# AI-multimodal/RankAAE

Hardware: AMD Instinct MI355X
Metric: training steps/sec (batch=256, 256-pt spectra) (higher is better)
Workload: dtype f32; 1 GPU; BASELINE configs[1]: 7000x256 synthetic spectra (7000 per GPU; train split 4900), batch 256/GPU, ae_form=compact, nstyle=6, n_aux=5, AdamW, 5 phases incl. smoothness; global_batch=256, parallelism=dp1, hip_graph=True, rng=philox tape (device), rccl_ranks=1

## Files before the change

### rankaae_amd/csrc/raae_common.h

```cpp
#pragma once
#include <hip/hip_runtime.h>
#include <stdint.h>
#include "../../include/rankaae_hip.h"

#define RAAE_WAVE 64

#define RAAE_CHECK_ARG(cond) do { if (!(cond)) return RAAE_EINVAL; } while (0)
#define RAAE_LAUNCH_RET() do { hipError_t e_ = hipGetLastError(); return (int)e_; } while (0)

typedef float f32x4 __attribute__((ext_vector_type(4)));

#ifdef RAAE_STAMPS
extern __device__ long long d_stamps[4][3][16];
extern __device__ unsigned long long d_stage_sum[4][3][16], d_stage_cnt[4][3][16];
extern __device__ long long d_stage_prev[4];
extern __device__ unsigned long long d_kind_sum[8][4][16], d_kind_cnt[8][4][16];
#endif
namespace raae {

__device__ __forceinline__ float wave_sum(float v) {
#pragma unroll
    for (int o = 32; o > 0; o >>= 1) v += __shfl_xor(v, o, 64);
    return v;
}
__device__ __forceinline__ double wave_sum(double v) {
#pragma unroll
    for (int o = 32; o > 0; o >>= 1) v += __shfl_xor(v, o, 64);
    return v;
}
__device__ __forceinline__ int wave_sum(int v) {
#pragma unroll
    for (int o = 32; o > 0; o >>= 1) v += __shfl_xor(v, o, 64);
    return v;
}

__device__ __forceinline__ double block_sum(double v, double* sh) {
    v = wave_sum(v);
    const int w = threadIdx.x >> 6, nw = (blockDim.x + 63) >> 6;
    __syncthreads();
    if ((threadIdx.x & 63) == 0) sh[w] = v;
    __syncthreads();
    double t = 0.0;
    for (int i = 0; i < nw; ++i) t += sh[i];
    return t;
}

__device__ __forceinline__ float prelu(float x, float a) { return x > 0.f ? x : a * x; }

__device__ __forceinline__ float softplus2(float x) {
    const float bx = 2.f * x;
    return bx > 20.f ? x : 0.5f * log1pf(expf(bx));
}

__device__ __forceinline__ void reduce_partials(const double* partials, int nparts, int C, double* tot_s,
                                                double* tot_q) {
    __shared__ double scr_s[256], scr_q[256];
    int Cp = 1;
    while (Cp < C) Cp <<= 1;
    const int J = 256 / Cp;
    const int t = threadIdx.x;
    if (t < 256) {
        const int c = t & (Cp - 1), j = t / Cp;
        double s = 0.0, q = 0.0;
        if (c < C) {
            const double2* p = reinterpret_cast<const double2*>(partials) + c;
            int i = j;
            for (; i + 3 * J < nparts; i += 4 * J) {
                const double2 v0 = p[(size_t)i * C], v1 = p[(size_t)(i + J) * C];
                const double2 v2 = p[(size_t)(i + 2 * J) * C], v3 = p[(size_t)(i + 3 * J) * C];
// ... 344 lines not shown
```

### rankaae_amd/csrc/raae_disc.hip

```cpp
#include "raae_common.h"
#include <stdlib.h>

namespace {

constexpr int DH = 64;
constexpr int DT = 16;
constexpr int DNS = 16;
constexpr int AP = DH + 1;

struct DiscArgs {
    const float* z_real; const float* styles; const float* noise; float sigma;
    const float* m1; const float* m2;
    const float* w1; const float* b1; const float* s1;
    const float* w2; const float* b2; const float* s2;
    const float* w3; const float* b3;
    const float* alpha;
    int n_real, n_fake, ns;
    float* dw1; float* db1; float* ds1; float* dw2; float* db2; float* ds2; float* dw3; float* db3;
    long slab_stride;
    float* dstyles;
    double* partial; unsigned* ticket; float* loss;
};

__device__ __forceinline__ double softplus_dd(double x) { return x > 0.0 ? x + log1p(exp(-x)) : log1p(exp(x)); }

template <bool MM>
__device__ __forceinline__ void disc_fused_body(const DiscArgs& a) {
    __shared__ float W1[DH * DNS], W2[DH * (DH + 1)], W3[DH], B1[DH], B2[DH], S1[DH], S2[DH];
    __shared__ float X[DT * DNS], Z1[DT * AP], A1[DT * AP], Z2[DT * AP], A2[DT * AP], G2[DT * AP], G1[DT * AP];
    __shared__ float DL[DT];
    __shared__ double shd[16];
    __shared__ unsigned s_last;
    const int t = threadIdx.x, ns = a.ns, n = a.n_real + a.n_fake;
    for (int i = t; i < DH * DNS; i += 256) { const int o = i / DNS, k = i - o * DNS; W1[i] = k < ns ? a.w1[o * ns + k] : 0.f; }
    for (int i = t; i < DH * DH; i += 256) { const int o = i >> 6, k = i & 63; W2[o * (DH + 1) + k] = a.w2[i]; }
    if (t < DH) { W3[t] = a.w3[t]; B1[t] = a.b1[t]; B2[t] = a.b2[t]; S1[t] = a.s1[t]; S2[t] = a.s2[t]; }
    const float b3 = a.b3[0];
    const float neg_alpha = -a.alpha[0];
    float aw2[16], aw1[4];
    f32x4 mw2[4];
#pragma unroll
    for (int i = 0; i < 4; ++i) mw2[i] = (f32x4){0.f, 0.f, 0.f, 0.f};
    const int lane = t & 63, wave = t >> 6, l15 = lane & 15, l4 = lane >> 4;
#pragma unroll
    for (int i = 0; i < 16; ++i) aw2[i] = 0.f;
#pragma unroll
    for (int i = 0; i < 4; ++i) aw1[i] = 0.f;
    float ab1 = 0.f, ab2 = 0.f, as1 = 0.f, as2 = 0.f, aw3 = 0.f, ab3 = 0.f;
    double lacc = 0.0;
    const int ntiles = (n + DT - 1) / DT;
    const int r4 = t >> 4, c4 = (t & 15) * 4;
    const int wo = t >> 2, wk = (t & 3) * 16;
    __syncthreads();
    for (int tile = blockIdx.x; tile < ntiles; tile += gridDim.x) {
        const int row0 = tile * DT;
        float m1v[4] = {1.f, 1.f, 1.f, 1.f}, m2v[4] = {1.f, 1.f, 1.f, 1.f};
        if (row0 + r4 < n) {
            if (a.m1) { const float4 v = *reinterpret_cast<const float4*>(a.m1 + (size_t)(row0 + r4) * DH + c4); m1v[0] = v.x; m1v[1] = v.y; m1v[2] = v.z; m1v[3] = v.w; }
            if (a.m2) { const float4 v = *reinterpret_cast<const float4*>(a.m2 + (size_t)(row0 + r4) * DH + c4); m2v[0] = v.x; m2v[1] = v.y; m2v[2] = v.z; m2v[3] = v.w; }
        }
        for (int i = t; i < DT * DNS; i += 256) {
            const int r = i / DNS, k = i - r * DNS, row = row0 + r;
            float v = 0.f;
            if (row < n && k < ns) {
                v = row < a.n_real ? a.z_real[(size_t)row * ns + k] : a.styles[(size_t)(row - a.n_real) * ns + k];
                if (a.noise) v += a.sigma * a.noise[(size_t)row * ns + k];
            }
            X[i] = v;
        }
        __syncthreads();
        {
            const int row = row0 + r4;
#pragma unroll
            for (int j = 0; j < 4; ++j) {
                const int o = c4 + j;
                float acc = B1[o];
                for (int k = 0; k < ns; ++k) acc = fmaf(X[r4 * DNS + k], W1[o * DNS + k], acc);
                Z1[r4 * AP + o] = acc;
                float v = acc > 0.f ? acc : acc * S1[o];
                v *= m1v[j];
                A1[r4 * AP + o] = row < n ? v : 0.f;
            }
        }
        __syncthreads();
        {
            const int row = row0 + r4;
            float acc[4] = {B2[c4], B2[c4 + 1], B2[c4 + 2], B2[c4 + 3]};
            if constexpr (MM) {
                f32x4 c = {0.f, 0.f, 0.f, 0.f};
                const float* pa = A1 + l15 * AP + l4;
                const float* pb = W2 + (16 * wave + l15) * (DH + 1) + l4;
#pragma unroll
                for (int q = 0; q < DH / 4; ++q) c = __builtin_amdgcn_mfma_f32_16x16x4f32(pa[4 * q], pb[4 * q], c, 0, 0, 0);
#pragma unroll
                for (int j = 0; j < 4; ++j) Z2[(4 * l4 + j) * AP + 16 * wave + l15] = c[j];
                __syncthreads();
#pragma unroll
                for (int j = 0; j < 4; ++j) acc[j] += Z2[r4 * AP + c4 + j];
            } else {
#pragma unroll 4
                for (int k = 0; k < DH; ++k) {
                    const float x = A1[r4 * AP + k];
#pragma unroll
                    for (int j = 0; j < 4; ++j) acc[j] = fmaf(x, W2[(c4 + j) * (DH + 1) + k], acc[j]);
                }
            }
#pragma unroll
            for (int j = 0; j < 4; ++j) {
                const int o = c4 + j;
                Z2[r4 * AP + o] = acc[j];
                float v = acc[j] > 0.f ? acc[j] : acc[j] * S2[o];
                v *= m2v[j];
                A2[r4 * AP + o] = row < n ? v : 0.f;
            }
        }
        __syncthreads();
        {
            float p = 0.f;
#pragma unroll
            for (int j = 0; j < 4; ++j) p = fmaf(A2[r4 * AP + c4 + j], W3[c4 + j], p);
            p += __shfl_xor(p, 1, 64); p += __shfl_xor(p, 2, 64); p += __shfl_xor(p, 4, 64); p += __shfl_xor(p, 8, 64);
            const int row = row0 + r4;
            if ((t & 15) == 0) {
                float d = 0.f;
                if (row < n) {
                    const float o = p + b3;
                    const float sg = 1.f / (1.f + expf(-o));
                    if (row < a.n_real) { lacc += softplus_dd(-(double)o) / (double)a.n_real; d = (sg - 1.f) / (float)a.n_real; }
                    else { lacc += softplus_dd((double)o) / (double)a.n_fake; d = sg / (float)a.n_fake; }
                }
                DL[r4] = d;
            }
        }
        __syncthreads();
        {
            const float d = DL[r4];
#pragma unroll
            for (int j = 0; j < 4; ++j) {
                const int o = c4 + j;
                float g = d * W3[o];
                g *= m2v[j];
                const float z = Z2[r4 * AP + o];
                G2[r4 * AP + o] = z > 0.f ? g : g * S2[o];
                Z2[r4 * AP + o] = z > 0.f ? 0.f : g * z;
            }
        }
        __syncthreads();
        if (t < DH) {
            float w = 0.f, b = 0.f, s = 0.f;
#pragma unroll 4
            for (int r = 0; r < DT; ++r) { w = fmaf(A2[r * AP + t], DL[r], w); b += G2[r * AP + t]; s += Z2[r * AP + t]; }
            aw3 += w; ab2 += b; as2 += s;
        }
        if (t == 64) { float b = 0.f; for (int r = 0; r < DT; ++r) b += DL[r]; ab3 += b; }
        if constexpr (MM) {
#pragma unroll
            for (int q = 0; q < DT / 4; ++q) {
                const float ga = G2[(4 * q + l4) * AP + 16 * wave + l15];
#pragma unroll
                for (int tk = 0; tk < 4; ++tk)
                    mw2[tk] = __builtin_amdgcn_mfma_f32_16x16x4f32(ga, A1[(4 * q + l4) * AP + 16 * tk + l15], mw2[tk], 0, 0, 0);
            }
        } else {
#pragma unroll 2
            for (int r = 0; r < DT; ++r) {
                const float g = G2[r * AP + wo];
#pragma unroll
                for (int j = 0; j < 16; ++j) aw2[j] = fmaf(g, A1[r * AP + wk + j], aw2[j]);
            }
        }
        {
            float acc[4] = {0.f, 0.f, 0.f, 0.f};
            if constexpr (MM) {
                f32x4 c = {0.f, 0.f, 0.f, 0.f};
                const float* pa = G2 + l15 * AP + l4;
                const float* pb = W2 + l4 * (DH + 1) + 16 * wave + l15;
#pragma unroll
                for (int q = 0; q < DH / 4; ++q)
                    c = __builtin_amdgcn_mfma_f32_16x16x4f32(pa[4 * q], pb[4 * q * (DH + 1)], c, 0, 0, 0);
#pragma unroll
                for (int j = 0; j < 4; ++j) G1[(4 * l4 + j) * AP + 16 * wave + l15] = c[j];
                __syncthreads();
#pragma unroll
                for (int j = 0; j < 4; ++j) acc[j] = G1[r4 * AP + c4 + j];
            } else {
#pragma unroll 4
                for (int o = 0; o < DH; ++o) {
                    const float g = G2[r4 * AP + o];
#pragma unroll
                    for (int j = 0; j < 4; ++j) acc[j] = fmaf(g, W2[o * (DH + 1) + c4 + j], acc[j]);
                }
            }
            __syncthreads();
#pragma unroll
            for (int j = 0; j < 4; ++j) {
                const int k = c4 + j;
                float g = acc[j];
                g *= m1v[j];
                const float z = Z1[r4 * AP + k];
                G1[r4 * AP + k] = z > 0.f ? g : g * S1[k];
                Z1[r4 * AP + k] = z > 0.f ? 0.f : g * z;
            }
        }
        __syncthreads();
        if (t < DH) {
            float b = 0.f, s = 0.f;
            for (int r = 0; r < DT; ++r) { b += G1[r * AP + t]; s += Z1[r * AP + t]; }
            ab1 += b; as1 += s;
        }
#pragma unroll
        for (int j = 0; j < 4; ++j) {
            const int idx = t + 256 * j;
            if (idx < DH * ns) {
                const int o = idx / ns, k = idx - o * ns;
                float w = 0.f;
#pragma unroll 4
                for (int r = 0; r < DT; ++r) w = fmaf(G1[r * AP + o], X[r * DNS + k], w);
                aw1[j] += w;
            }
        }
        for (int i = t; i < DT * ns; i += 256) {
            const int r = i / ns, k = i - r * ns, row = row0 + r;
            if (row >= a.n_real && row < n) {
                float d = 0.f;
#pragma unroll 4
                for (int o = 0; o < DH; ++o) d = fmaf(G1[r * AP + o], W1[o * DNS + k], d);
                a.dstyles[(size_t)(row - a.n_real) * ns + k] = neg_alpha * d;
            }
        }
        __syncthreads();
    }
    const size_t slab = (size_t)blockIdx.x * (size_t)a.slab_stride;
    if constexpr (MM) {
#pragma unroll
        for (int tk = 0; tk < 4; ++tk)
#pragma unroll
            for (int j = 0; j < 4; ++j) a.dw2[slab + (16 * wave + 4 * l4 + j) * DH + 16 * tk + l15] = mw2[tk][j];
    } else {
#pragma unroll
        for (int j = 0; j < 16; ++j) a.dw2[slab + wo * DH + wk + j] = aw2[j];
    }
#pragma unroll
    for (int j = 0; j < 4; ++j) { const int idx = t + 256 * j; if (idx < DH * ns) a.dw1[slab + idx] = aw1[j]; }
    if (t < DH) {
        a.db1[slab + t] = ab1; a.ds1[slab + t] = as1; a.db2[slab + t] = ab2; a.ds2[slab + t] = as2; a.dw3[slab + t] = aw3;
    }
    if (t == 64) a.db3[slab] = ab3;
    const double tot = raae::block_sum(lacc, shd);
    if (t == 0) {
        a.partial[blockIdx.x] = tot;
        __threadfence();
        s_last = atomicAdd(a.ticket, 1u) == gridDim.x - 1 ? 1u : 0u;
    }
    __syncthreads();
    if (s_last) {
        __threadfence();
        double sum = 0.0;
        for (unsigned i = t; i < gridDim.x; i += 256) sum += ((volatile double*)a.partial)[i];
        sum = raae::block_sum(sum, shd);
        if (t == 0) {
            a.loss[0] = (float)sum;
            *a.ticket = 0u;
        }
    }
}
template <bool MM>
__global__ __launch_bounds__(256) void disc_fused_kernel(DiscArgs a) { disc_fused_body<MM>(a); }
template <bool MM>
__global__ __launch_bounds__(256) void disc_fused_kernel_m(const DiscArgs* t) {
    const DiscArgs a = t[blockIdx.z];
    disc_fused_body<MM>(a);
}

}

extern "C" int raae_disc_fused(const raae_disc_fused_t* in, int* nslab, void* stream) {
    RAAE_CHECK_ARG(in && in->z_real && in->styles && in->w1 && in->b1 && in->s1 && in->w2 && in->b2 && in->s2 && in->w3 &&
                   in->b3 && in->alpha && in->n_real > 0 && in->n_fake > 0 && in->ns >= 1 && in->ns <= DNS);
    RAAE_CHECK_ARG(in->hidden == DH && in->dw1 && in->db1 && in->ds1 && in->dw2 && in->db2 && in->ds2 && in->dw3 && in->db3 &&
                   in->dstyles && in->partial && in->ticket && in->loss);
    DiscArgs a;
    a.z_real = in->z_real; a.styles = in->styles; a.noise = in->noise; a.sigma = in->sigma; a.m1 = in->mask1; a.m2 = in->mask2;
    a.w1 = in->w1; a.b1 = in->b1; a.s1 = in->s1; a.w2 = in->w2; a.b2 = in->b2; a.s2 = in->s2; a.w3 = in->w3; a.b3 = in->b3;
    a.alpha = in->alpha; a.n_real = in->n_real; a.n_fake = in->n_fake; a.ns = in->ns;
    a.dw1 = in->dw1; a.db1 = in->db1; a.ds1 = in->ds1; a.dw2 = in->dw2; a.db2 = in->db2; a.ds2 = in->ds2;
    a.dw3 = in->dw3; a.db3 = in->db3; a.slab_stride = in->slab_stride; a.dstyles = in->dstyles;
    a.partial = in->partial; a.ticket = in->ticket; a.loss = in->loss;
    const int ntiles = (in->n_real + in->n_fake + DT - 1) / DT;
    const int grid = ntiles < 256 ? ntiles : 256;
    if (nslab) *nslab = grid;
    static const int force = [] { const char* e = getenv("RAAE_DISC_MFMA"); return e ? atoi(e) : -1; }();
    const bool mm = force >= 0 ? force != 0 : (in->n_real + in->n_fake >= 2048);
    if (mm) raae::launch(disc_fused_kernel<true>, disc_fused_kernel_m<true>, dim3(grid), dim3(256), 0, (hipStream_t)stream, a);
    else raae::launch(disc_fused_kernel<false>, disc_fused_kernel_m<false>, dim3(grid), dim3(256), 0, (hipStream_t)stream, a);
    RAAE_LAUNCH_RET();
}
```

### rankaae_amd/csrc/raae_loss.hip

```cpp
#include "raae_common.h"

namespace {

struct StyleFwdArgs { const float* z; int B; int C; raae_bn_t bn; float* out; };
__device__ __forceinline__ void style_bn_fwd_body(const float* z, int B, int C, const raae_bn_t& bn, float* out) {
    __shared__ float s_mean[64], s_rstd[64];
    raae::bn_prologue(bn, C, s_mean, s_rstd, blockIdx.x == 0);
    const long n = (long)B * C;
    for (long i = (long)blockIdx.x * 256 + threadIdx.x; i < n; i += (long)gridDim.x * 256) {
        const int c = (int)(i % C);
        out[i] = (z[i] - s_mean[c]) * s_rstd[c];
    }
}

__global__ __launch_bounds__(256) void style_bn_fwd_kernel(StyleFwdArgs a) { style_bn_fwd_body(a.z, a.B, a.C, a.bn, a.out); }
__global__ __launch_bounds__(256) void style_bn_fwd_kernel_m(const StyleFwdArgs* t) {
    const StyleFwdArgs a = t[blockIdx.z];
    style_bn_fwd_body(a.z, a.B, a.C, a.bn, a.out);
}

struct StyleBwdArgs { const float* dy; const float* y; int B; int C; raae_bn_t bn; float scale; float* dz; };
__device__ __forceinline__ void style_bn_bwd_body(const float* dy, const float* y, int B, int C,
                                                  const raae_bn_t& bn, float scale, float* dz) {
    __shared__ float s_mean[64], s_rstd[64];
    __shared__ double s_s[64], s_q[64];
    __shared__ double red[2][1024];
    raae::bn_prologue(bn, C, s_mean, s_rstd, false);
    const int tid = threadIdx.x;
    const int nphase = 1024 / C;
    const int c = tid % C, ph = tid / C;
    double s = 0.0, q = 0.0;
    if (ph < nphase) {
        int r = ph;
        for (; r + 3 * nphase < B; r += 4 * nphase) {
            float g[4], yv[4];
#pragma unroll
            for (int u = 0; u < 4; ++u) { g[u] = dy[(size_t)(r + u * nphase) * C + c]; yv[u] = y[(size_t)(r + u * nphase) * C + c]; }
#pragma unroll
            for (int u = 0; u < 4; ++u) { const float gg = scale * g[u]; s += (double)gg; q += (double)gg * (double)yv[u]; }
        }
        for (; r < B; r += nphase) {
            const float g = scale * dy[(size_t)r * C + c];
            s += (double)g;
            q += (double)g * (double)y[(size_t)r * C + c];
        }
    }
    red[0][tid] = s; red[1][tid] = q;
    __syncthreads();
    __shared__ double red2[2][64 * 8];
    if (tid < C * 8) {
        const int cc = tid >> 3, part = tid & 7;
        double ts = 0.0, tq = 0.0;
        for (int p = part; p < nphase; p += 8) { ts += red[0][p * C + cc]; tq += red[1][p * C + cc]; }
// ... 580 lines not shown
    if (fin && fin->ticket) { f.scale = fin->scale; f.out = fin->out; f.slot = fin->slot; f.acc_slot = fin->acc_slot; f.ticket = fin->ticket; }
    return f;
}

struct ReconArgs { const float* x; const float* y; int B; int L; int scale; double* partial; float* dy; LossFin fin; };
__device__ __forceinline__ void recon_body(const float* x, const float* y, int B, int L, int scale,
                                           double* partial, float* dy, const LossFin& fin) {
    __shared__ double shd[16];
    const int lane = threadIdx.x & 63, wv = threadIdx.x >> 6;
    double acc = 0.0;
    for (int row = blockIdx.x * 4 + wv; row < B; row += gridDim.x * 4) {
        const float* xr = x + (size_t)row * L;
        const float* yr = y + (size_t)row * L;
        float c = 1.f, gscale = 0.f;
        if (scale) {
            float sx = 0.f, sy = 0.f;
            for (int l = lane; l < L; l += 64) { sx += xr[l]; sy += yr[l]; }
            sx = raae::wave_sum(sx); sy = raae::wave_sum(sy);
            const float mx = sx / (float)L, my = sy / (float)L;
            const float r = fabsf(my) / fabsf(mx);
            c = fminf(fmaxf(r, 0.7f), 1.3f);
            if (lane == 0) acc += 0.1 * (double)(r - 1.f) * (double)(r - 1.f) / (double)B;
            const float sg = my > 0.f ? 1.f : (my < 0.f ? -1.f : 0.f);
            gscale = 0.2f * (r - 1.f) * sg / (fabsf(mx) * (float)L * (float)B);
        }
        const float inv = 1.f / ((float)B * (float)L);
        float se = 0.f;
        for (int l = lane; l < L; l += 64) {
            const float e = yr[l] - xr[l] * c;
            se += e * e;
            if (dy) dy[(size_t)row * L + l] = 2.f * e * inv + gscale;
        }
        se = raae::wave_sum(se);
        if (lane == 0) acc += (double)se / ((double)B * (double)L);
    }
    const double t = raae::block_sum(acc, shd);
    if (threadIdx.x == 0) partial[blockIdx.x] = t;
    loss_fin_last_block(fin, partial);
}

__global__ __launch_bounds__(256) void recon_kernel(ReconArgs a) { recon_body(a.x, a.y, a.B, a.L, a.scale, a.partial, a.dy, a.fin); }
__global__ __launch_bounds__(256) void recon_kernel_m(const ReconArgs* t) {
    const ReconArgs a = t[blockIdx.z];
    recon_body(a.x, a.y, a.B, a.L, a.scale, a.partial, a.dy, a.fin);
}

#define SM_MAXT 33
struct Taps { float w[SM_MAXT]; int n; };

struct SmoothArgs { const float* x; int B; int L; Taps tp; double* partial; float* dx; LossFin fin; };
template <int NT>
__device__ __forceinline__ void smooth_body(const float* x, int B, int L, const Taps& tp, double* partial, float* dx, const LossFin& fin) {
    const int ntap = NT > 0 ? NT : tp.n;
    extern __shared__ __attribute__((aligned(16))) float smem[];
    __shared__ double shd[16];
    const int lane = threadIdx.x & 63, wv = threadIdx.x >> 6;
    float* xs = smem + (size_t)wv * 2 * L;
    float* es = xs + L;
    const int half = (ntap - 1) / 2;
    double acc = 0.0;
    const float inv = 1.f / ((float)B * (float)L);
    for (int row = blockIdx.x * 4 + wv; row < B; row += gridDim.x * 4) {
        const float* xr = x + (size_t)row * L;
        for (int l = lane; l < L; l += 64) xs[l] = xr[l];
        __builtin_amdgcn_wave_barrier();
        float se = 0.f;
        for (int l = lane; l < L; l += 64) {
            float g = 0.f;
#pragma unroll
            for (int t = 0; t < ntap; ++t) {
                int j = l + t - half;
                j = j < 0 ? 0 : (j > L - 1 ? L - 1 : j);
                g += tp.w[t] * xs[j];
            }
            const float e = xs[l] - g;
            es[l] = e;
            se += e * e;
        }
        se = raae::wave_sum(se);
        if (lane == 0) acc += (double)se / ((double)B * (double)L);
        __builtin_amdgcn_wave_barrier();
        if (dx) {
            for (int j = lane; j < L; j += 64) {
                float gt = 0.f;
#pragma unroll
                for (int t = 0; t < ntap; ++t) {
                    const int l = j - t + half;
                    if (l >= 0 && l < L) gt += tp.w[t] * es[l];
                }
                if (j == 0) {
                    for (int l = 0; l < half && l < L; ++l)
                        for (int t = 0; t < half - l; ++t) gt += tp.w[t] * es[l];
                }
                if (j == L - 1) {
                    for (int l = max(0, L - half); l < L; ++l)
                        for (int t = L - l + half; t < ntap; ++t) gt += tp.w[t] * es[l];
                }
                dx[(size_t)row * L + j] = 2.f * inv * (es[j] - gt);
            }
        }
        __builtin_amdgcn_wave_barrier();
    }
    const double t = raae::block_sum(acc, shd);
    if (threadIdx.x == 0) partial[blockIdx.x] = t;
    loss_fin_last_block(fin, partial);
}

template <int NT>
__global__ __launch_bounds__(256) void smooth_kernel(SmoothArgs a) { smooth_body<NT>(a.x, a.B, a.L, a.tp, a.partial, a.dx, a.fin); }
template <int NT>
__global__ __launch_bounds__(256) void smooth_kernel_m(const SmoothArgs* t) {
    __shared__ SmoothArgs slot;
    const SmoothArgs& a = raae::args_from_table(&slot, t);
    smooth_body<NT>(a.x, a.B, a.L, a.tp, a.partial, a.dx, a.fin);
}

struct MseArgs { const float* a; const float* b; long n; double* partial; float* da; LossFin fin; };
__device__ __forceinline__ void mse_body(const float* a, const float* b, long n, double* partial, float* da, const LossFin& fin) {
    __shared__ double shd[16];
    double acc = 0.0;
    const float inv = 1.f / (float)n;
    for (long i = (long)blockIdx.x * 256 + threadIdx.x; i < n; i += (long)gridDim.x * 256) {
        const float e = a[i] - b[i];
        acc += (double)e * (double)e;
        if (da) da[i] = 2.f * e * inv;
    }
    const double t = raae::block_sum(acc, shd);
    if (threadIdx.x == 0) partial[blockIdx.x] = t / (double)n;
    loss_fin_last_block(fin, partial);
}

__global__ __launch_bounds__(256) void mse_kernel(MseArgs a) { mse_body(a.a, a.b, a.n, a.partial, a.da, a.fin); }
__global__ __launch_bounds__(256) void mse_kernel_m(const MseArgs* t) {
    const MseArgs a = t[blockIdx.z];
    mse_body(a.a, a.b, a.n, a.partial, a.da, a.fin);
}

__device__ __forceinline__ double softplus_d(double x) { return x > 0.0 ? x + log1p(exp(-x)) : log1p(exp(x)); }

struct BceArgs { const float* o; int n_real; int n_fake; float* loss; float* d; };
__device__ __forceinline__ void bce_pair_body(const float* o, int n_real, int n_fake, float* loss, float* d) {
    __shared__ double shd[16];
    double acc = 0.0;
    for (int i = threadIdx.x; i < n_real + n_fake; i += 1024) {
        const float v = o[i];
        const float sg = 1.f / (1.f + expf(-v));
        if (i < n_real) { acc += softplus_d(-(double)v) / (double)n_real; if (d) d[i] = (sg - 1.f) / (float)n_real; }
        else { acc += softplus_d((double)v) / (double)n_fake; if (d) d[i] = sg / (float)n_fake; }
    }
    const double t = raae::block_sum(acc, shd);
    if (threadIdx.x == 0) loss[0] = (float)t;
}

__global__ __launch_bounds__(1024) void bce_pair_kernel(BceArgs a) { bce_pair_body(a.o, a.n_real, a.n_fake, a.loss, a.d); }
__global__ __launch_bounds__(1024) void bce_pair_kernel_m(const BceArgs* t) {
    const BceArgs a = t[blockIdx.z];
    bce_pair_body(a.o, a.n_real, a.n_fake, a.loss, a.d);
}
// ... 312 lines not shown
```

### rankaae_amd/csrc/raae_optim.hip

```cpp
#include "raae_common.h"
#include "raae_philox.h"
#include <string.h>
#include <stdlib.h>

namespace {

#include "raae_optim_body.inc"

template <int RULE, bool WIDE, bool CHK, bool SC>
__global__ __launch_bounds__(256) void update_kernel(UpdateArgs a) { update_body<RULE, WIDE, CHK, SC>(a, blockIdx.x, gridDim.x); }
template <int RULE, bool WIDE, bool CHK, bool SC>
__global__ __launch_bounds__(256) void update_kernel_m(const UpdateArgs* t) {
    const UpdateArgs a = t[blockIdx.z];
    update_body<RULE, WIDE, CHK, SC>(a, blockIdx.x, gridDim.x);
}
struct UpdateInst { void (*single)(UpdateArgs); void (*multi)(const UpdateArgs*); };
#define RAAE_UPD(R, W, C, S) {update_kernel<R, W, C, S>, update_kernel_m<R, W, C, S>}
#define RAAE_UPD_SHAPE(R, W) {{RAAE_UPD(R, W, false, false), RAAE_UPD(R, W, false, true)},                            \
                              {RAAE_UPD(R, W, true, false), RAAE_UPD(R, W, true, true)}}
#define RAAE_UPD_RULE(R) {RAAE_UPD_SHAPE(R, false), RAAE_UPD_SHAPE(R, true)}
const UpdateInst kUpdate[4][2][2][2] = {RAAE_UPD_RULE(RAAE_OPT_ADAM), RAAE_UPD_RULE(RAAE_OPT_ADAM),
                                        RAAE_UPD_RULE(RAAE_OPT_RADAM), RAAE_UPD_RULE(RAAE_OPT_ADABOUND)};
#undef RAAE_UPD_RULE
#undef RAAE_UPD_SHAPE
#undef RAAE_UPD

inline bool optim_wide(int max_nslab) { return max_nslab > 16; }
inline dim3 optim_grid(long n, int max_nslab, long cap = 4096) {
    long g = optim_wide(max_nslab) ? (n + 31) / 32 : (n + 255) / 256;
    if (g > cap) g = cap;
    return dim3((int)g);
}

constexpr int GRAD_NORM_PARTS = RAAE_GRAD_NORM_PARTS;
struct GradNormArgs { const float* g_slabs; long slab_stride; const unsigned short* seg_nslab; long n; double max_norm;
                      double* partial; unsigned* ticket; float* out; int* clipped; };
template <bool WIDE>
__device__ __forceinline__ void grad_norm_body(const GradNormArgs& a) {
    __shared__ double s_red[16];
    __shared__ unsigned s_last;
    double acc = 0.0;
    for_each_grad<WIDE, false>(a.g_slabs, a.slab_stride, a.seg_nslab, a.n, blockIdx.x, gridDim.x,
                               [&](long, float g) { acc += (double)g * (double)g; });
    const double part = raae::block_sum(acc, s_red);
    if (threadIdx.x == 0) {
        a.partial[blockIdx.x] = part;
        __threadfence();
        s_last = atomicAdd(a.ticket, 1u) == gridDim.x - 1 ? 1u : 0u;
    }
    __syncthreads();
    if (!s_last) return;
    __threadfence();
    double t = 0.0;
    for (unsigned i = threadIdx.x; i < gridDim.x; i += 256) t += ((volatile double*)a.partial)[i];
    t = raae::block_sum(t, s_red);
    if (threadIdx.x == 0) {
// ... 13 lines not shown
}

struct SlabReduceArgs { const float* g_slabs; long slab_stride; const unsigned short* seg_nslab; long n; float* out; };
template <bool WIDE>
__device__ __forceinline__ void slab_reduce_body(const SlabReduceArgs& a) {
    for_each_grad<WIDE, true>(a.g_slabs, a.slab_stride, a.seg_nslab, a.n, blockIdx.x, gridDim.x,
                              [&](long i, float g) { a.out[i] = g; });
}
template <bool WIDE> __global__ __launch_bounds__(256) void slab_reduce_kernel(SlabReduceArgs a) { slab_reduce_body<WIDE>(a); }
template <bool WIDE> __global__ __launch_bounds__(256) void slab_reduce_kernel_m(const SlabReduceArgs* t) {
    const SlabReduceArgs a = t[blockIdx.z];
    slab_reduce_body<WIDE>(a);
}

struct EmaArgs { float* ema; const float* p; long n; float d; float omd; };
__device__ __forceinline__ void ema_body(const EmaArgs& a) {
    const long nthreads = (long)gridDim.x * 256, t0 = (long)blockIdx.x * 256 + threadIdx.x;
    const float d = a.d, omd = a.omd;
    if ((((uintptr_t)a.ema | (uintptr_t)a.p) & 15) == 0) {
        const long nq = a.n >> 2;
        float4* e4 = reinterpret_cast<float4*>(a.ema);
        const float4* p4 = reinterpret_cast<const float4*>(a.p);
        for (long q = t0; q < nq; q += nthreads) {
            float4 e = e4[q];
            const float4 w = p4[q];
            e.x = fmaf(d, e.x, omd * w.x); e.y = fmaf(d, e.y, omd * w.y);
            e.z = fmaf(d, e.z, omd * w.z); e.w = fmaf(d, e.w, omd * w.w);
            e4[q] = e;
        }
        const long i = (nq << 2) + t0;
        if (i < a.n) a.ema[i] = fmaf(d, a.ema[i], omd * a.p[i]);
    } else {
        for (long i = t0; i < a.n; i += nthreads) a.ema[i] = fmaf(d, a.ema[i], omd * a.p[i]);
    }
}
__global__ __launch_bounds__(256) void ema_kernel(EmaArgs a) { ema_body(a); }
__global__ __launch_bounds__(256) void ema_kernel_m(const EmaArgs* t) {
    const EmaArgs a = t[blockIdx.z];
    ema_body(a);
}

__global__ void tick_kernel(int* steps, int n, unsigned mask, unsigned long long* rng_counter, int* cursor,
                            int cursor_inc) {
    if (blockIdx.x == 0 && threadIdx.x == 0) {
        for (int i = 0; i < n; ++i) if (mask & (1u << i)) steps[i] += 1;
        if (rng_counter) {
            rng_counter[0] += 1ull;
            raae::mask_keys_store(rng_counter, rng_counter[1], rng_counter[0]);
        }
        if (cursor) cursor[0] += cursor_inc;
    }
}

__device__ __forceinline__ void fill_quad(float* tape, const int* seg_desc, const float* seg_scale, int nseg, long total,
                                          unsigned long long seed, unsigned long long ctr, long q) {
    const long e0 = q * 4;
    int lo = 0, hi = nseg - 1;
    while (lo < hi) {
        const int mid = (lo + hi + 1) >> 1;
        if ((long)seg_desc[mid * 4] <= e0) lo = mid; else hi = mid - 1;
    }
    const int kind = seg_desc[lo * 4 + 2];
    const long send = (long)seg_desc[lo * 4] + seg_desc[lo * 4 + 1];
    float o[4];
    if (kind == 0) {
        raae::normal4(((long)seg_desc[lo * 4 + 3] + (e0 - seg_desc[lo * 4])) >> 2, ctr, seed, o);
    } else if (kind == 1) {
        const raae::MaskGen g = raae::mask_gen_make(seed, ctr, (uint32_t)seg_desc[lo * 4 + 3], seg_scale[lo]);
#pragma unroll
        for (int j = 0; j < 4; ++j) o[j] = raae::mask_val(g, (uint32_t)(e0 + j - seg_desc[lo * 4]));
    } else {
        const raae::MaskGen g = raae::mask_gen_make(seed, ctr, (uint32_t)seg_desc[lo * 4 + 3], seg_scale[lo]);
#pragma unroll
        for (int j = 0; j < 4; ++j) {
            const uint32_t e = 2u * (uint32_t)(e0 + j - seg_desc[lo * 4]);
            const uint32_t lo16 = raae::mask_keep(g, e) ? 0x3F80u : 0u, hi16 = raae::mask_keep(g, e + 1u) ? 0x3F80u : 0u;
            o[j] = __uint_as_float(lo16 | (hi16 << 16));
        }
    }
#pragma unroll
    for (int j = 0; j < 4; ++j) if (e0 + j < send && e0 + j < total) tape[e0 + j] = o[j];
}

struct RngFillArgs { float* tape; const int* seg_desc; const float* seg_scale; int nseg; long total; unsigned long long seed;
                     const unsigned long long* counter; };
__device__ __forceinline__ void rng_fill_body(const RngFillArgs& a) {
    const unsigned long long ctr = a.counter ? a.counter[0] : 0ull;
    for (long q = (long)blockIdx.x * 256 + threadIdx.x; q * 4 < a.total; q += (long)gridDim.x * 256)
        fill_quad(a.tape, a.seg_desc, a.seg_scale, a.nseg, a.total, a.seed, ctr, q);
}
__global__ __launch_bounds__(256) void rng_fill_kernel(RngFillArgs a) { rng_fill_body(a); }
__global__ __launch_bounds__(256) void rng_fill_kernel_m(const RngFillArgs* t) {
    const RngFillArgs a = t[blockIdx.z];
    rng_fill_body(a);
}

struct StepBeginArgs {
    int* steps; int nsteps; unsigned step_mask; unsigned long long* rng_state; int* cursor; int stride; unsigned* ticket;
    const float* spec; const float* aux; const long* idx; int B; int L; int n_aux; float spec_noise;
    const float* noise_tape;
    long noise_goff;
    float* spec_out; float* aux_out;
    float* tape; const int* seg_desc; const float* seg_scale; int nseg; long total;
};
__device__ __forceinline__ void step_begin_body(const StepBeginArgs& a) {
    __shared__ unsigned long long s_ctr, s_seed;
    __shared__ int s_cur;
    unsigned my_ticket = 0u;
    if (threadIdx.x == 0) {
        s_ctr = a.rng_state[0] + 1ull;
        s_seed = a.rng_state[1];
        s_cur = a.cursor[0] + a.stride;
        __threadfence();
        my_ticket = atomicAdd(a.ticket, 1u);
    }
    __syncthreads();
    const unsigned long long ctr = s_ctr, seed = s_seed;
    const int cur = s_cur;
    const long* idx = a.idx + (cur - a.B);
    const long nthreads = (long)gridDim.x * 256, t0 = (long)blockIdx.x * 256 + threadIdx.x;
    const long n = (long)a.B * a.L;
    if ((a.L & 3) == 0) {
        for (long i4 = t0; i4 * 4 < n; i4 += nthreads) {
            const long i = i4 * 4;
            const int b = (int)(i / a.L), l = (int)(i - (long)b * a.L);
            float4 v = *reinterpret_cast<const float4*>(a.spec + (size_t)idx[b] * a.L + l);
            if (a.spec_noise != 0.f) {
                float z[4];
                if (a.noise_tape != nullptr) { const float4 t = *reinterpret_cast<const float4*>(a.noise_tape + i); z[0] = t.x; z[1] = t.y; z[2] = t.z; z[3] = t.w; }
                else raae::normal4((a.noise_goff + i) >> 2, ctr, seed, z);
                v.x += z[0] * a.spec_noise; v.y += z[1] * a.spec_noise; v.z += z[2] * a.spec_noise; v.w += z[3] * a.spec_noise;
            }
            *reinterpret_cast<float4*>(a.spec_out + i) = v;
        }
    } else {
        for (long i = t0; i < n; i += nthreads) {
            const int b = (int)(i / a.L), l = (int)(i - (long)b * a.L);
            float v = a.spec[(size_t)idx[b] * a.L + l];
            if (a.spec_noise != 0.f) {
                if (a.noise_tape != nullptr) v += a.noise_tape[i] * a.spec_noise;
                else { float z[4]; raae::normal4((a.noise_goff + i) >> 2, ctr, seed, z); v += z[(a.noise_goff + i) & 3] * a.spec_noise; }
            }
            a.spec_out[i] = v;
        }
    }
    const long na = (long)a.B * a.n_aux;
    for (long i = t0; i < na; i += nthreads) {
        const int b = (int)(i / a.n_aux), k = (int)(i - (long)b * a.n_aux);
        a.aux_out[i] = a.aux[(size_t)idx[b] * a.n_aux + k];
    }
    if (a.nseg > 0) {
        __shared__ int s_desc[4 * 256];
        __shared__ float s_scale[256];
        const int* desc = a.seg_desc;
        const float* scale = a.seg_scale;
        if (a.nseg <= 256) {
            for (int i = threadIdx.x; i < 4 * a.nseg; i += 256) s_desc[i] = a.seg_desc[i];
            for (int i = threadIdx.x; i < a.nseg; i += 256) s_scale[i] = a.seg_scale[i];
            __syncthreads();
            desc = s_desc; scale = s_scale;
        }
        for (long q = t0; q * 4 < a.total; q += nthreads)
            fill_quad(a.tape, desc, scale, a.nseg, a.total, seed, ctr, q);
    }
    if (threadIdx.x == 0 && my_ticket == gridDim.x - 1) {
        for (int i = 0; i < a.nsteps; ++i) if (a.step_mask & (1u << i)) a.steps[i] += 1;
        a.rng_state[0] = ctr;
        raae::mask_keys_store(a.rng_state, seed, ctr);
        a.cursor[0] = cur;
        *a.ticket = 0u;
    }
}
__global__ __launch_bounds__(256) void step_begin_kernel(StepBeginArgs a) { step_begin_body(a); }
__global__ __launch_bounds__(256) void step_begin_kernel_m(const StepBeginArgs* t) {
    const StepBeginArgs a = t[blockIdx.z];
    step_begin_body(a);
}

}

extern "C" int raae_optim_step_clip(float* p, float* m, float* v, const float* g_slabs, long slab_stride,
                                    const unsigned short* seg_nslab, long n, int rule, const double* hyper, const int* step,
                                    int max_nslab, int* nan_step, const float* scale, void* stream) {
    RAAE_CHECK_ARG(rule >= RAAE_OPT_ADAM && rule <= RAAE_OPT_ADABOUND);
    RAAE_CHECK_ARG(p && m && v && g_slabs && seg_nslab && hyper && step && n > 0 && (n % 64) == 0 && max_nslab >= 0);
    const UpdateArgs a = {p, m, v, g_slabs, slab_stride, seg_nslab, n, hyper, step, rule == RAAE_OPT_ADAMW, scale, nan_step};
    const UpdateInst& k = kUpdate[rule][optim_wide(max_nslab)][nan_step != nullptr][scale != nullptr];
    raae::launch(k.single, k.multi, optim_grid(n, max_nslab), dim3(256), 0, (hipStream_t)stream, a);
    RAAE_LAUNCH_RET();
}

extern "C" int raae_optim_step_chk(float* p, float* m, float* v, const float* g_slabs, long slab_stride,
                                   const unsigned short* seg_nslab, long n, int rule, const double* hyper, const int* step,
                                   int max_nslab, int* nan_step, void* stream) {
    RAAE_CHECK_ARG(nan_step);
    return raae_optim_step_clip(p, m, v, g_slabs, slab_stride, seg_nslab, n, rule, hyper, step, max_nslab, nan_step, nullptr, stream);
}

extern "C" int raae_optim_step(float* p, float* m, float* v, const float* g_slabs, long slab_stride,
                               const unsigned short* seg_nslab, long n, int rule, const double* hyper, const int* step,
                               int max_nslab, void* stream) {
    return raae_optim_step_clip(p, m, v, g_slabs, slab_stride, seg_nslab, n, rule, hyper, step, max_nslab, nullptr, nullptr, stream);
}

extern "C" int raae_adam_step(float* p, float* m, float* v, const float* g_slabs, long slab_stride,
                              const unsigned short* seg_nslab, long n, const double* hyper, const int* step,
                              int decoupled, int max_nslab, void* stream) {
    return raae_optim_step(p, m, v, g_slabs, slab_stride, seg_nslab, n, decoupled ? RAAE_OPT_ADAMW : RAAE_OPT_ADAM, hyper, step,
                           max_nslab, stream);
}

extern "C" int raae_grad_norm(const float* g_slabs, long slab_stride, const unsigned short* seg_nslab, long n, int max_nslab,
                              double max_norm, double* partial, unsigned* ticket, float* out, int* clipped, void* stream) {
    RAAE_CHECK_ARG(g_slabs && seg_nslab && partial && ticket && out && clipped && n > 0 && (n % 64) == 0 && max_nslab >= 0);
    RAAE_CHECK_ARG(max_norm > 0.0 && max_norm <= 1.7976931348623157e308);
    const GradNormArgs a = {g_slabs, slab_stride, seg_nslab, n, max_norm, partial, ticket, out, clipped};
    const dim3 grid = optim_grid(n, max_nslab, GRAD_NORM_PARTS);
    if (optim_wide(max_nslab)) raae::launch(grad_norm_kernel<true>, grad_norm_kernel_m<true>, grid, dim3(256), 0, (hipStream_t)stream, a);
    else raae::launch(grad_norm_kernel<false>, grad_norm_kernel_m<false>, grid, dim3(256), 0, (hipStream_t)stream, a);
    RAAE_LAUNCH_RET();
}

extern "C" int raae_slab_reduce(const float* g_slabs, long slab_stride, const unsigned short* seg_nslab, long n,
                                float* out, int max_nslab, void* stream) {
// ... 220 lines not shown
```

Measured before the change: 829.6 steps/s (five-phase steps on 256-row batches, summed over ranks).

## Prefetch first tiles early, reorder step-begin RNG fill, unroll smoothness boundary taps

The discriminator kernel now issues the first tile's input and mask loads before staging the weights into shared memory, so their latency overlaps the weight staging. The step-begin kernel stages segment descriptors up front, runs the RNG tape fill first with an incremental segment lookup, and issues the first gathered spectrum and aux loads during that fill. The smoothness backward kernel turns its tap loop into branchless selects and unrolls the edge corrections when the tap count is known at compile time. Debug timestamp macros are added but compile to nothing by default; the changes add register pressure and code complexity.

```diff
diff --git a/rankaae_amd/csrc/raae_common.h b/rankaae_amd/csrc/raae_common.h
--- a/rankaae_amd/csrc/raae_common.h
+++ b/rankaae_amd/csrc/raae_common.h
@@ -15,6 +15,21 @@
 extern __device__ unsigned long long d_stage_sum[4][3][16], d_stage_cnt[4][3][16];
 extern __device__ long long d_stage_prev[4];
 extern __device__ unsigned long long d_kind_sum[8][4][16], d_kind_cnt[8][4][16];
+#define RAAE_LSTAMP_DEFINE(NAME) \
+    __device__ unsigned long long d_##NAME##_sum[16], d_##NAME##_cnt[16]; __device__ long long d_##NAME##_prev; \
+    extern "C" int raae_debug_##NAME##_stamps(unsigned long long* sum, unsigned long long* cnt) { \
+        hipError_t e = hipMemcpyFromSymbol(sum, HIP_SYMBOL(d_##NAME##_sum), sizeof(unsigned long long) * 16); \
+        if (e != hipSuccess) return (int)e; \
+        return (int)hipMemcpyFromSymbol(cnt, HIP_SYMBOL(d_##NAME##_cnt), sizeof(unsigned long long) * 16); }
+#define LSTAMP_W(NAME, i) do { if (blockIdx.x == 0 && threadIdx.x == 0) { \
+        const long long now_ = wall_clock64(); \
+        if ((i) > 0) { d_##NAME##_sum[i] += (unsigned long long)(now_ - d_##NAME##_prev); d_##NAME##_cnt[i] += 1ull; } \
+        d_##NAME##_prev = now_; } } while (0)
+#define LSTAMP(NAME, i) do { __syncthreads(); LSTAMP_W(NAME, i); } while (0)
+#else
+#define RAAE_LSTAMP_DEFINE(NAME)
+#define LSTAMP_W(NAME, i) do { } while (0)
+#define LSTAMP(NAME, i) do { } while (0)
 #endif
 namespace raae {
 
diff --git a/rankaae_amd/csrc/raae_disc.hip b/rankaae_amd/csrc/raae_disc.hip
--- a/rankaae_amd/csrc/raae_disc.hip
+++ b/rankaae_amd/csrc/raae_disc.hip
@@ -1,5 +1,8 @@
 #include "raae_common.h"
 #include <stdlib.h>
+
+RAAE_LSTAMP_DEFINE(disc)
+#define DSTAMP(i) do { if constexpr (!MM) LSTAMP(disc, i); } while (0)
 
 namespace {
 
@@ -32,6 +35,25 @@
     __shared__ double shd[16];
     __shared__ unsigned s_last;
     const int t = threadIdx.x, ns = a.ns, n = a.n_real + a.n_fake;
+    DSTAMP(0);
+    static_assert(DT * DNS == 256, "one input element per thread");
+    const int r4 = t >> 4, c4 = (t & 15) * 4;
+    float m1v[4], m2v[4], xin;
+    auto tile_loads = [&](int row0) {
+#pragma unroll
+        for (int j = 0; j < 4; ++j) { m1v[j] = 1.f; m2v[j] = 1.f; }
+        if (row0 + r4 < n) {
+            if (a.m1) { const float4 v = *reinterpret_cast<const float4*>(a.m1 + (size_t)(row0 + r4) * DH + c4); m1v[0] = v.x; m1v[1] = v.y; m1v[2] = v.z; m1v[3] = v.w; }
+            if (a.m2) { const float4 v = *reinterpret_cast<const float4*>(a.m2 + (size_t)(row0 + r4) * DH + c4); m2v[0] = v.x; m2v[1] = v.y; m2v[2] = v.z; m2v[3] = v.w; }
+        }
+        const int r = t / DNS, k = t - r * DNS, row = row0 + r;
+        xin = 0.f;
+        if (row < n && k < ns) {
+            xin = row < a.n_real ? a.z_real[(size_t)row * ns + k] : a.styles[(size_t)(row - a.n_real) * ns + k];
+            if (a.noise) xin += a.sigma * a.noise[(size_t)row * ns + k];
+        }
+    };
+    tile_loads((int)blockIdx.x * DT);
     for (int i = t; i < DH * DNS; i += 256) { const int o = i / DNS, k = i - o * DNS; W1[i] = k < ns ? a.w1[o * ns + k] : 0.f; }
     for (int i = t; i < DH * DH; i += 256) { const int o = i >> 6, k = i & 63; W2[o * (DH + 1) + k] = a.w2[i]; }
     if (t < DH) { W3[t] = a.w3[t]; B1[t] = a.b1[t]; B2[t] = a.b2[t]; S1[t] = a.s1[t]; S2[t] = a.s2[t]; }
@@ -49,26 +71,18 @@
     float ab1 = 0.f, ab2 = 0.f, as1 = 0.f, as2 = 0.f, aw3 = 0.f, ab3 = 0.f;
     double lacc = 0.0;
     const int ntiles = (n + DT - 1) / DT;
-    const int r4 = t >> 4, c4 = (t & 15) * 4;
     const int wo = t >> 2, wk = (t & 3) * 16;
+    X[t] = xin;
     __syncthreads();
+    DSTAMP(1);
     for (int tile = blockIdx.x; tile < ntiles; tile += gridDim.x) {
         const int row0 = tile * DT;
-        float m1v[4] = {1.f, 1.f, 1.f, 1.f}, m2v[4] = {1.f, 1.f, 1.f, 1.f};
-        if (row0 + r4 < n) {
-            if (a.m1) { const float4 v = *reinterpret_cast<const float4*>(a.m1 + (size_t)(row0 + r4) * DH + c4); m1v[0] = v.x; m1v[1] = v.y; m1v[2] = v.z; m1v[3] = v.w; }
-            if (a.m2) { const float4 v = *reinterpret_cast<const float4*>(a.m2 + (size_t)(row0 + r4) * DH + c4); m2v[0] = v.x; m2v[1] = v.y; m2v[2] = v.z; m2v[3] = v.w; }
-        }
-        for (int i = t; i < DT * DNS; i += 256) {
-            const int r = i / DNS, k = i - r * DNS, row = row0 + r;
-            float v = 0.f;
-            if (row < n && k < ns) {
-                v = row < a.n_real ? a.z_real[(size_t)row * ns + k] : a.styles[(size_t)(row - a.n_real) * ns + k];
-                if (a.noise) v += a.sigma * a.noise[(size_t)row * ns + k];
-            }
-            X[i] = v;
-        }
-        __syncthreads();
+        if (tile != (int)blockIdx.x) {
+            tile_loads(row0);
+            X[t] = xin;
+            __syncthreads();
+        }
+        DSTAMP(2);
         {
             const int row = row0 + r4;
 #pragma unroll
@@ -83,6 +97,7 @@
             }
         }
         __syncthreads();
+        DSTAMP(3);
         {
             const int row = row0 + r4;
             float acc[4] = {B2[c4], B2[c4 + 1], B2[c4 + 2], B2[c4 + 3]};
@@ -115,6 +130,7 @@
             }
         }
         __syncthreads();
+        DSTAMP(4);
         {
             float p = 0.f;
 #pragma unroll
@@ -133,6 +149,7 @@
             }
         }
         __syncthreads();
+        DSTAMP(5);
         {
             const float d = DL[r4];
 #pragma unroll
@@ -146,6 +163,7 @@
             }
         }
         __syncthreads();
+        DSTAMP(6);
         if (t < DH) {
             float w = 0.f, b = 0.f, s = 0.f;
 #pragma unroll 4
@@ -153,6 +171,7 @@
             aw3 += w; ab2 += b; as2 += s;
         }
         if (t == 64) { float b = 0.f; for (int r = 0; r < DT; ++r) b += DL[r]; ab3 += b; }
+        DSTAMP(7);
         if constexpr (MM) {
 #pragma unroll
             for (int q = 0; q < DT / 4; ++q) {
@@ -169,6 +188,7 @@
                 for (int j = 0; j < 16; ++j) aw2[j] = fmaf(g, A1[r * AP + wk + j], aw2[j]);
             }
         }
+        DSTAMP(8);
         {
             float acc[4] = {0.f, 0.f, 0.f, 0.f};
             if constexpr (MM) {
@@ -203,11 +223,13 @@
             }
         }
         __syncthreads();
+        DSTAMP(9);
         if (t < DH) {
             float b = 0.f, s = 0.f;
             for (int r = 0; r < DT; ++r) { b += G1[r * AP + t]; s += Z1[r * AP + t]; }
             ab1 += b; as1 += s;
         }
+        DSTAMP(10);
 #pragma unroll
         for (int j = 0; j < 4; ++j) {
             const int idx = t + 256 * j;
@@ -219,6 +241,7 @@
                 aw1[j] += w;
             }
         }
+        DSTAMP(11);
         for (int i = t; i < DT * ns; i += 256) {
             const int r = i / ns, k = i - r * ns, row = row0 + r;
             if (row >= a.n_real && row < n) {
@@ -230,6 +253,7 @@
         }
         __syncthreads();
     }
+    DSTAMP(12);
     const size_t slab = (size_t)blockIdx.x * (size_t)a.slab_stride;
     if constexpr (MM) {
 #pragma unroll
@@ -246,6 +270,7 @@
         a.db1[slab + t] = ab1; a.ds1[slab + t] = as1; a.db2[slab + t] = ab2; a.ds2[slab + t] = as2; a.dw3[slab + t] = aw3;
     }
     if (t == 64) a.db3[slab] = ab3;
+    DSTAMP(13);
     const double tot = raae::block_sum(lacc, shd);
     if (t == 0) {
         a.partial[blockIdx.x] = tot;
@@ -253,6 +278,7 @@
         s_last = atomicAdd(a.ticket, 1u) == gridDim.x - 1 ? 1u : 0u;
     }
     __syncthreads();
+    DSTAMP(14);
     if (s_last) {
         __threadfence();
         double sum = 0.0;
@@ -263,6 +289,7 @@
             *a.ticket = 0u;
         }
     }
+    DSTAMP(15);
 }
 template <bool MM>
 __global__ __launch_bounds__(256) void disc_fused_kernel(DiscArgs a) { disc_fused_body<MM>(a); }
diff --git a/rankaae_amd/csrc/raae_loss.hip b/rankaae_amd/csrc/raae_loss.hip
--- a/rankaae_amd/csrc/raae_loss.hip
+++ b/rankaae_amd/csrc/raae_loss.hip
@@ -1,4 +1,7 @@
 #include "raae_common.h"
+
+RAAE_LSTAMP_DEFINE(smooth)
+#define SSTAMP(i) do { if constexpr (NT == 17) LSTAMP_W(smooth, i); } while (0)
 
 namespace {
 
@@ -685,6 +688,7 @@
 template <int NT>
 __device__ __forceinline__ void smooth_body(const float* x, int B, int L, const Taps& tp, double* partial, float* dx, const LossFin& fin) {
     const int ntap = NT > 0 ? NT : tp.n;
+    SSTAMP(0);
     extern __shared__ __attribute__((aligned(16))) float smem[];
     __shared__ double shd[16];
     const int lane = threadIdx.x & 63, wv = threadIdx.x >> 6;
@@ -697,6 +701,7 @@
         const float* xr = x + (size_t)row * L;
         for (int l = lane; l < L; l += 64) xs[l] = xr[l];
         __builtin_amdgcn_wave_barrier();
+        SSTAMP(1);
         float se = 0.f;
         for (int l = lane; l < L; l += 64) {
             float g = 0.f;
@@ -713,30 +718,61 @@
         se = raae::wave_sum(se);
         if (lane == 0) acc += (double)se / ((double)B * (double)L);
         __builtin_amdgcn_wave_barrier();
+        SSTAMP(2);
         if (dx) {
             for (int j = lane; j < L; j += 64) {
                 float gt = 0.f;
 #pragma unroll
                 for (int t = 0; t < ntap; ++t) {
                     const int l = j - t + half;
-                    if (l >= 0 && l < L) gt += tp.w[t] * es[l];
+                    const bool in = l >= 0 && l < L;
+                    const float nx = gt + tp.w[t] * es[in ? l : j];
+                    gt = in ? nx : gt;
                 }
-                if (j == 0) {
-                    for (int l = 0; l < half && l < L; ++l)
-                        for (int t = 0; t < half - l; ++t) gt += tp.w[t] * es[l];
-                }
-                if (j == L - 1) {
-                    for (int l = max(0, L - half); l < L; ++l)
-                        for (int t = L - l + half; t < ntap; ++t) gt += tp.w[t] * es[l];
+                if constexpr (NT > 0) {
+                    constexpr int HF = (NT - 1) / 2;
+                    if (j == 0) {
+#pragma unroll
+                        for (int l = 0; l < HF; ++l) {
+                            if (l < L) {
+                                const float e = es[l];
+#pragma unroll
+                                for (int t = 0; t < HF - l; ++t) gt += tp.w[t] * e;
+                            }
+                        }
+                    }
+                    if (j == L - 1) {
+#pragma unroll
+                        for (int u = 0; u < HF; ++u) {
+                            const int l = L - HF + u;
+                            if (l >= 0) {
+                                const float e = es[l];
+#pragma unroll
+                                for (int t = 2 * HF - u; t < NT; ++t) gt += tp.w[t] * e;
+                            }
+                        }
+                    }
+                } else {
+                    if (j == 0) {
+                        for (int l = 0; l < half && l < L; ++l)
+                            for (int t = 0; t < half - l; ++t) gt += tp.w[t] * es[l];
+                    }
+                    if (j == L - 1) {
+                        for (int l = max(0, L - half); l < L; ++l)
+                            for (int t = L - l + half; t < ntap; ++t) gt += tp.w[t] * es[l];
+                    }
                 }
                 dx[(size_t)row * L + j] = 2.f * inv * (es[j] - gt);
             }
         }
         __builtin_amdgcn_wave_barrier();
+        SSTAMP(3);
     }
     const double t = raae::block_sum(acc, shd);
     if (threadIdx.x == 0) partial[blockIdx.x] = t;
+    SSTAMP(4);
     loss_fin_last_block(fin, partial);
+    SSTAMP(5);
 }
 
 template <int NT>
diff --git a/rankaae_amd/csrc/raae_optim.hip b/rankaae_amd/csrc/raae_optim.hip
--- a/rankaae_amd/csrc/raae_optim.hip
+++ b/rankaae_amd/csrc/raae_optim.hip
@@ -2,6 +2,8 @@
 #include "raae_philox.h"
 #include <string.h>
 #include <stdlib.h>
+
+RAAE_LSTAMP_DEFINE(head)
 
 namespace {
 
@@ -121,14 +123,16 @@
     }
 }
 
-__device__ __forceinline__ void fill_quad(float* tape, const int* seg_desc, const float* seg_scale, int nseg, long total,
-                                          unsigned long long seed, unsigned long long ctr, long q) {
-    const long e0 = q * 4;
-    int lo = 0, hi = nseg - 1;
+__device__ __forceinline__ int fill_seg_find(const int* seg_desc, int lo, int hi, long e0) {
     while (lo < hi) {
         const int mid = (lo + hi + 1) >> 1;
         if ((long)seg_desc[mid * 4] <= e0) lo = mid; else hi = mid - 1;
     }
+    return lo;
+}
+__device__ __forceinline__ void fill_quad_in(float* tape, const int* seg_desc, const float* seg_scale, int lo, long total,
+                                             unsigned long long seed, unsigned long long ctr, long q) {
+    const long e0 = q * 4;
     const int kind = seg_desc[lo * 4 + 2];
     const long send = (long)seg_desc[lo * 4] + seg_desc[lo * 4 + 1];
     float o[4];
@@ -150,6 +154,10 @@
 #pragma unroll
     for (int j = 0; j < 4; ++j) if (e0 + j < send && e0 + j < total) tape[e0 + j] = o[j];
 }
+__device__ __forceinline__ void fill_quad(float* tape, const int* seg_desc, const float* seg_scale, int nseg, long total,
+                                          unsigned long long seed, unsigned long long ctr, long q) {
+    fill_quad_in(tape, seg_desc, seg_scale, fill_seg_find(seg_desc, 0, nseg - 1, q * 4), total, seed, ctr, q);
+}
 
 struct RngFillArgs { float* tape; const int* seg_desc; const float* seg_scale; int nseg; long total; unsigned long long seed;
                      const unsigned long long* counter; };
@@ -175,7 +183,15 @@
 __device__ __forceinline__ void step_begin_body(const StepBeginArgs& a) {
     __shared__ unsigned long long s_ctr, s_seed;
     __shared__ int s_cur;
+    __shared__ int s_desc[4 * 256];
+    __shared__ float s_scale[256];
     unsigned my_ticket = 0u;
+    LSTAMP_W(head, 0);
+    const bool staged = a.nseg > 0 && a.nseg <= 256;
+    if (staged) {
+        for (int i = threadIdx.x; i < 4 * a.nseg; i += 256) s_desc[i] = a.seg_desc[i];
+        for (int i = threadIdx.x; i < a.nseg; i += 256) s_scale[i] = a.seg_scale[i];
+    }
     if (threadIdx.x == 0) {
         s_ctr = a.rng_state[0] + 1ull;
         s_seed = a.rng_state[1];
@@ -184,28 +200,78 @@
         my_ticket = atomicAdd(a.ticket, 1u);
     }
     __syncthreads();
+    LSTAMP_W(head, 1);
     const unsigned long long ctr = s_ctr, seed = s_seed;
     const int cur = s_cur;
     const long* idx = a.idx + (cur - a.B);
     const long nthreads = (long)gridDim.x * 256, t0 = (long)blockIdx.x * 256 + threadIdx.x;
-    const long n = (long)a.B * a.L;
-    if ((a.L & 3) == 0) {
+    const long n = (long)a.B * a.L, na = (long)a.B * a.n_aux;
+    const bool vec = (a.L & 3) == 0;
+    const long gi = vec ? t0 * 4 : t0;
+    const bool g_on = gi < n, x_on = t0 < na;
+    long grow = 0, xrow = 0;
+    int gl = 0, xk = 0;
+    if (g_on) { const int b = (int)(gi / a.L); gl = (int)(gi - (long)b * a.L); grow = idx[b]; }
+    if (x_on) { const int b = (int)(t0 / a.n_aux); xk = (int)(t0 - (long)b * a.n_aux); xrow = idx[b]; }
+    float4 gv = make_float4(0.f, 0.f, 0.f, 0.f);
+    float xv = 0.f;
+    bool requested = false;
+    auto request_rows = [&]() {
+        if (g_on) {
+            if (vec) gv = *reinterpret_cast<const float4*>(a.spec + (size_t)grow * a.L + gl);
+            else gv.x = a.spec[(size_t)grow * a.L + gl];
+        }
+        if (x_on) xv = a.aux[(size_t)xrow * a.n_aux + xk];
+        requested = true;
+    };
+    LSTAMP(head, 2);
+    if (a.nseg > 0) {
+        const int* desc = staged ? s_desc : a.seg_desc;
+        const float* scale = staged ? s_scale : a.seg_scale;
+        int lo = 0;
+        bool first = true;
+        for (long q = t0; q * 4 < a.total; q += nthreads) {
+            const long e0 = q * 4;
+            if (first) { lo = fill_seg_find(desc, 0, a.nseg - 1, e0); first = false; }
+            else {
+                int w = 0;
+                while (w < 4 && lo + 1 < a.nseg && (long)desc[(lo + 1) * 4] <= e0) { ++lo; ++w; }
+                if (w == 4) lo = fill_seg_find(desc, lo, a.nseg - 1, e0);
+            }
+            fill_quad_in(a.tape, desc, scale, lo, a.total, seed, ctr, q);
+            if (!requested) request_rows();
+        }
+    }
+    if (!requested) request_rows();
+    LSTAMP(head, 3);
+    if (vec) {
+        bool pre = true;
         for (long i4 = t0; i4 * 4 < n; i4 += nthreads) {
             const long i = i4 * 4;
-            const int b = (int)(i / a.L), l = (int)(i - (long)b * a.L);
-            float4 v = *reinterpret_cast<const float4*>(a.spec + (size_t)idx[b] * a.L + l);
-            if (a.spec_noise != 0.f) {
-                float z[4];
+            const bool noisy = a.spec_noise != 0.f;
+            float z[4] = {0.f, 0.f, 0.f, 0.f};
+            if (noisy) {
                 if (a.noise_tape != nullptr) { const float4 t = *reinterpret_cast<const float4*>(a.noise_tape + i); z[0] = t.x; z[1] = t.y; z[2] = t.z; z[3] = t.w; }
                 else raae::normal4((a.noise_goff + i) >> 2, ctr, seed, z);
-                v.x += z[0] * a.spec_noise; v.y += z[1] * a.spec_noise; v.z += z[2] * a.spec_noise; v.w += z[3] * a.spec_noise;
-            }
+            }
+            float4 v;
+            if (pre) { v = gv; pre = false; }
+            else {
+                const int b = (int)(i / a.L), l = (int)(i - (long)b * a.L);
+                v = *reinterpret_cast<const float4*>(a.spec + (size_t)idx[b] * a.L + l);
+            }
+            if (noisy) { v.x += z[0] * a.spec_noise; v.y += z[1] * a.spec_noise; v.z += z[2] * a.spec_noise; v.w += z[3] * a.spec_noise; }
             *reinterpret_cast<float4*>(a.spec_out + i) = v;
         }
     } else {
+        bool pre = true;
         for (long i = t0; i < n; i += nthreads) {
-            const int b = (int)(i / a.L), l = (int)(i - (long)b * a.L);
-            float v = a.spec[(size_t)idx[b] * a.L + l];
+            float v;
+            if (pre) { v = gv.x; pre = false; }
+            else {
+                const int b = (int)(i / a.L), l = (int)(i - (long)b * a.L);
+                v = a.spec[(size_t)idx[b] * a.L + l];
+            }
             if (a.spec_noise != 0.f) {
                 if (a.noise_tape != nullptr) v += a.noise_tape[i] * a.spec_noise;
                 else { float z[4]; raae::normal4((a.noise_goff + i) >> 2, ctr, seed, z); v += z[(a.noise_goff + i) & 3] * a.spec_noise; }
@@ -213,25 +279,20 @@
             a.spec_out[i] = v;
         }
     }
-    const long na = (long)a.B * a.n_aux;
-    for (long i = t0; i < na; i += nthreads) {
-        const int b = (int)(i / a.n_aux), k = (int)(i - (long)b * a.n_aux);
-        a.aux_out[i] = a.aux[(size_t)idx[b] * a.n_aux + k];
-    }
-    if (a.nseg > 0) {
-        __shared__ int s_desc[4 * 256];
-        __shared__ float s_scale[256];
-        const int* desc = a.seg_desc;
-        const float* scale = a.seg_scale;
-        if (a.nseg <= 256) {
-            for (int i = threadIdx.x; i < 4 * a.nseg; i += 256) s_desc[i] = a.seg_desc[i];
-            for (int i = threadIdx.x; i < a.nseg; i += 256) s_scale[i] = a.seg_scale[i];
-            __syncthreads();
-            desc = s_desc; scale = s_scale;
-        }
-        for (long q = t0; q * 4 < a.total; q += nthreads)
-            fill_quad(a.tape, desc, scale, a.nseg, a.total, seed, ctr, q);
-    }
+    LSTAMP(head, 4);
+    {
+        bool pre = true;
+        for (long i = t0; i < na; i += nthreads) {
+            float v;
+            if (pre) { v = xv; pre = false; }
+            else {
+                const int b = (int)(i / a.n_aux), k = (int)(i - (long)b * a.n_aux);
+                v = a.aux[(size_t)idx[b] * a.n_aux + k];
+            }
+            a.aux_out[i] = v;
+        }
+    }
+    LSTAMP(head, 5);
     if (threadIdx.x == 0 && my_ticket == gridDim.x - 1) {
         for (int i = 0; i < a.nsteps; ++i) if (a.step_mask & (1u << i)) a.steps[i] += 1;
         a.rng_state[0] = ctr;
@@ -239,6 +300,7 @@
         a.cursor[0] = cur;
         *a.ticket = 0u;
     }
+    LSTAMP_W(head, 6);
 }
 __global__ __launch_bounds__(256) void step_begin_kernel(StepBeginArgs a) { step_begin_body(a); }
 __global__ __launch_bounds__(256) void step_begin_kernel_m(const StepBeginArgs* t) {
```

Result: no change. 830.3 steps/s (five-phase steps on 256-row batches, summed over ranks) (median of 3 runs) (+0.1%).
